# sieste/greb-climate-model

Measured on AMD Instinct MI355X. Metric: simulated-years/sec at 96x48 grid (ensemble aggregate); diffusion HBM GB/s vs roofline, higher is better.
Workload: dtype f32; 1 GPU; 96x48 GREB ensemble, 512 members/GPU x 1 GPU, CO2 sweep 280-1120 ppm, 32 scenario years after 1 flux-correction year, dt=12h, dt_crcl=0.5h; members_per_gpu=512, arithmetic=fast, gather=none (1 GPU)

## Files before the change

greb_climate_model_amd/csrc/greb_member.hip:

```cpp
#include <cstdlib>

#include "greb_kernels.h"
#include "greb_pair.h"
#include "greb_physics_step.h"
#include "greb_stencil.h"

namespace greb {

constexpr int NX = 96, NY = 48, NQ = 24, NP = 4608;
constexpr int kThreads = 512;
constexpr int RS = 2 * NX + 16;
constexpr int XB = (NY + 2) * RS;
constexpr int kOffX = RS;
constexpr int kOffW = 2 * XB + RS;
constexpr int kOffWX = 3 * XB;
constexpr int kOffWY = kOffWX + NP;
constexpr int kOffRowK = kOffWY + NP;
constexpr int kRowKCsDif = 7;
constexpr int kLdsFloats = kOffRowK + NY * kRowKWords;
constexpr size_t kLdsBytes = (size_t)kLdsFloats * sizeof(float);

bool member_layout_supported(const RowTables& t, int nx, int ny) {
  if (nx != NX || ny != NY) return false;
  for (int k = 0; k < NY; ++k) {
    const bool sub = (k <= 9 || k >= 38);
    if ((t.subcycled[k] != 0) != sub) return false;
    const bool chain = (k == 0 || k == NY - 1);
    if ((t.dif_time2[k] > 1 || t.adv_time2[k] > 1) != chain) return false;
  }
  if (t.dif_time2[0] != t.dif_time2[NY - 1] || t.adv_time2[0] != t.adv_time2[NY - 1]) return false;
  return true;
}

__device__ __forceinline__ f4 comp(const q8& q, int tr) {
  return tr == 0 ? f4{{q.v[0].x, q.v[1].x, q.v[2].x, q.v[3].x}} : f4{{q.v[0].y, q.v[1].y, q.v[2].y, q.v[3].y}};
}
__device__ __forceinline__ q8 zip(const f4& a, const f4& b) {
  q8 r;
#pragma unroll
  for (int i = 0; i < 4; ++i) r.v[i] = v2{a.v[i], b.v[i]};
  return r;
}

struct TaskAddr { int c, l, r, kq; };

__device__ __forceinline__ q8 ld8p(const lfloat* p) {
  const vfloat4 a = *(const __attribute__((address_space(3))) vfloat4*)p;
  const vfloat4 b = *(const __attribute__((address_space(3))) vfloat4*)(p + kHalfRow);
  q8 r;
  r.v[0] = v2{a.x, a.y}; r.v[1] = v2{a.z, a.w}; r.v[2] = v2{b.x, b.y}; r.v[3] = v2{b.z, b.w};
  return r;
}

template <bool SUB>
__device__ __forceinline__ q8 fast_row(const q8& LT, const q8& CT, const q8& RT, const q8& Tm2, const q8& Tm1, const q8& Tp1,
                                       const q8& Tp2, const q8& LW, const q8& CW, const q8& RW, const q8& Wm2, const q8& Wm1,
                                       const q8& Wp1, const q8& Wp2, const f4& xq, const f4& yq, bool last_quad,
                                       float cs_dif, float dif_ccy, bool calm_q) {
  v2 T[12], w[12];
#pragma unroll
  for (int j = 0; j < 4; ++j) {
    T[j] = LT.v[j]; T[4 + j] = CT.v[j]; T[8 + j] = RT.v[j];
    w[j] = LW.v[j]; w[4 + j] = CW.v[j]; w[8 + j] = RW.v[j];
  }
  float um[4], up[4], vm[4], vp[4];
#pragma unroll
  for (int i = 0; i < 4; ++i) {
    split_sign(xq.v[i], um[i], up[i]);
    split_sign(yq.v[i], vm[i], vp[i]);
  }
  return substep_pair<SUB>(T, w, Tm2, Tm1, Tp1, Tp2, Wm2, Wm1, Wp1, Wp2, um, up, vm, vp, cs_dif, dif_ccy, last_quad, calm_q);
}

__device__ __forceinline__ void st8p(lfloat* o, const q8& xn) {
  vfloat4 a, b;
  a.x = xn.v[0].x; a.y = xn.v[0].y; a.z = xn.v[1].x; a.w = xn.v[1].y;
  b.x = xn.v[2].x; b.y = xn.v[2].y; b.z = xn.v[3].x; b.w = xn.v[3].y;
  *(__attribute__((address_space(3))) vfloat4*)o = a;
  *(__attribute__((address_space(3))) vfloat4*)(o + kHalfRow) = b;
}

__device__ __forceinline__ q8 strict_row(const q8& LT, const q8& CT, const q8& RT, const q8& Tm2, const q8& Tm1, const q8& Tp1,
                                         const q8& Tp2, const q8& LW, const q8& CW, const q8& RW, const q8& Wm2, const q8& Wm1,
                                         const q8& Wp1, const q8& Wp2, const f4& xq, const f4& yq, int k, int q,
                                         const RowK& rk, bool calm_q) {
#pragma clang fp contract(off)
  q8 xn;
  v2 T[12], w[12];
#pragma unroll
  for (int j = 0; j < 4; ++j) {
    T[j] = LT.v[j]; T[4 + j] = CT.v[j]; T[8 + j] = RT.v[j];
    w[j] = LW.v[j]; w[4 + j] = CW.v[j]; w[8 + j] = RW.v[j];
  }
  v2 dTx[4], dTy[4], dd[4], da[4];
  dif_lon_strict(T, w, rk.dif_cc, dTx);
  if (rk.sub) {
    v2 T1h[4] = {T[4], T[5], T[6], T[7]};
    clamp_add(T1h, dTx);
#pragma unroll
    for (int i = 0; i < 4; ++i) dTx[i] = T1h[i] - T[4 + i];
  }
  dif_lat_strict(CT, Tm1, Tp1, Wm1, Wp1, rk.dif_ccy, k, NY, dTy);
#pragma unroll
  for (int i = 0; i < 4; ++i) dd[i] = CW.v[i] * (dTx[i] + dTy[i]);
  if (!rk.sub) {
    adv_lon_full_strict(T, w, xq.v, rk.adv_cc, dTx);
  } else {
    v2 T1h[4] = {T[4], T[5], T[6], T[7]};
    adv_lon_sub_strict(T, w, xq.v, rk.adv_cc, q == NQ - 1, dTx);
    clamp_add(T1h, dTx);
#pragma unroll
    for (int i = 0; i < 4; ++i) dTx[i] = T1h[i] - T[4 + i];
  }
  adv_lat_strict(CT, Tm2, Tm1, Tp1, Tp2, Wm2, Wm1, Wp1, Wp2, yq.v, rk.adv_ccy, k, NY, dTy);
#pragma unroll
  for (int i = 0; i < 4; ++i) {
    da[i] = dTx[i] + dTy[i];
    const v2 xd = T[4 + i] + dd[i];
    v2 x = xd + da[i];
    if (calm_q) x.y = xd.y;
    xn.v[i] = x;
  }
  return xn;
}

template <bool STRICT, bool SUB>
__device__ __forceinline__ q8 one_row(const q8& LT, const q8& CT, const q8& RT, const q8& Tm2, const q8& Tm1, const q8& Tp1,
                                      const q8& Tp2, const q8& LW, const q8& CW, const q8& RW, const q8& Wm2, const q8& Wm1,
                                      const q8& Wp1, const q8& Wp2, const f4& xq, const f4& yq, int k, int q, const RowK& rk,
                                      bool calm_q) {
  if (STRICT) return strict_row(LT, CT, RT, Tm2, Tm1, Tp1, Tp2, LW, CW, RW, Wm2, Wm1, Wp1, Wp2, xq, yq, k, q, rk, calm_q);
  return fast_row<SUB>(LT, CT, RT, Tm2, Tm1, Tp1, Tp2, LW, CW, RW, Wm2, Wm1, Wp1, Wp2, xq, yq, q == NQ - 1, rk.dif_cc, rk.dif_ccy,
                       calm_q);
}

template <bool STRICT>
__device__ __forceinline__ RowK task_consts(const lfloat* lds, int k, float ccy_dif) {
  if (STRICT) return row_consts((const lfloat*)(lds + kOffRowK), k);
  RowK rk{};
  rk.dif_cc = lds[kOffRowK + k * kRowKWords + kRowKCsDif];
  rk.dif_ccy = ccy_dif;
  return rk;
}

template <bool STRICT, bool SUB>
__device__ __forceinline__ void row_task(lfloat* lds, int cur, const TaskAddr& ta, float ccy_dif, bool calm_q = false) {
  const int k = ta.kq & 255, q = ta.kq >> 8;
  const lfloat* Xc = lds + kOffX + cur * XB;
  const lfloat* Wc = lds + kOffW;
  const RowK rk = task_consts<STRICT>(lds, k, ccy_dif);
  const f4 xq = ld4(lds + kOffWX + k * NX + 4 * q), yq = ld4(lds + kOffWY + k * NX + 4 * q);
  const lfloat* xb = Xc + ta.c - 2 * RS;
  const lfloat* wb = Wc + ta.c - 2 * RS;
  const q8 Tm2 = ld8p(xb), Tm1 = ld8p(xb + RS), CT = ld8p(xb + 2 * RS), Tp1 = ld8p(xb + 3 * RS), Tp2 = ld8p(xb + 4 * RS);
  const q8 Wm2 = ld8p(wb), Wm1 = ld8p(wb + RS), CW = ld8p(wb + 2 * RS), Wp1 = ld8p(wb + 3 * RS), Wp2 = ld8p(wb + 4 * RS);
  const q8 LT = ld8p(Xc + ta.l), RT = ld8p(Xc + ta.r), LW = ld8p(Wc + ta.l), RW = ld8p(Wc + ta.r);
  const q8 xn = one_row<STRICT, SUB>(LT, CT, RT, Tm2, Tm1, Tp1, Tp2, LW, CW, RW, Wm2, Wm1, Wp1, Wp2, xq, yq, k, q, rk, calm_q);
  st8p(lds + kOffX + (cur ^ 1) * XB + ta.c, xn);
}

template <bool STRICT, bool SUB>
__device__ __forceinline__ void row_task2(lfloat* lds, int cur, const TaskAddr& ta, float ccy_dif, bool calm_q = false) {
  const int k = ta.kq & 255, q = ta.kq >> 8;
  const lfloat* Xc = lds + kOffX + cur * XB;
  const lfloat* Wc = lds + kOffW;
  const lfloat* xb = Xc + ta.c - 2 * RS;
  const lfloat* wb = Wc + ta.c - 2 * RS;
  const q8 T0 = ld8p(xb), T1 = ld8p(xb + RS), T2 = ld8p(xb + 2 * RS), T3 = ld8p(xb + 3 * RS), T4 = ld8p(xb + 4 * RS);
  const q8 W0 = ld8p(wb), W1 = ld8p(wb + RS), W2 = ld8p(wb + 2 * RS), W3 = ld8p(wb + 3 * RS), W4 = ld8p(wb + 4 * RS);
  lfloat* out = lds + kOffX + (cur ^ 1) * XB + ta.c;
  {
    const q8 LT = ld8p(Xc + ta.l), RT = ld8p(Xc + ta.r), LW = ld8p(Wc + ta.l), RW = ld8p(Wc + ta.r);
    const f4 xq = ld4(lds + kOffWX + k * NX + 4 * q), yq = ld4(lds + kOffWY + k * NX + 4 * q);
    const RowK rk = task_consts<STRICT>(lds, k, ccy_dif);
    st8p(out, one_row<STRICT, SUB>(LT, T2, RT, T0, T1, T3, T4, LW, W2, RW, W0, W1, W3, W4, xq, yq, k, q, rk, calm_q));
  }
  __builtin_amdgcn_sched_barrier(0);
  {
    const q8 T5 = ld8p(xb + 5 * RS), W5 = ld8p(wb + 5 * RS);
    const q8 LT = ld8p(Xc + ta.l + RS), RT = ld8p(Xc + ta.r + RS), LW = ld8p(Wc + ta.l + RS), RW = ld8p(Wc + ta.r + RS);
    const f4 xq = ld4(lds + kOffWX + (k + 1) * NX + 4 * q), yq = ld4(lds + kOffWY + (k + 1) * NX + 4 * q);
    const RowK rk = task_consts<STRICT>(lds, k + 1, ccy_dif);
    st8p(out + RS, one_row<STRICT, SUB>(LT, T3, RT, T1, T2, T4, T5, LW, W3, RW, W1, W2, W4, W5, xq, yq, k + 1, q, rk, calm_q));
  }
}

struct BulkTasks { TaskAddr t[3]; };

enum { kNone = 0, kS1 = 1, kF1 = 2, kST = 3, kFT = 4 };
struct Pass { int kind, index; };
__host__ __device__ constexpr Pass deal_fast(int wave, int i) {
  constexpr Pass none{kNone, 0};
#if defined(GREB_TUNING) && defined(GREB_DEAL_FAST)
  constexpr Pass t[8][3] = {GREB_DEAL_FAST};
#else
  constexpr Pass t[8][3] = {
       {{kST, 0}, {kF1, 0}, none},      {{kST, 2}, {kF1, 1}, none},
       {{kFT, 1}, {kF1, 3}, none},      {{kFT, 2}, {kS1, 0}, {kF1, 2}},
       {{kST, 1}, none, none},          {{kFT, 0}, none, none},
       {none, none, none},              {{kF1, 4}, none, none}};
#endif
  return t[wave][i];
}
__host__ __device__ constexpr Pass deal_strict(int wave, int i) {
  constexpr Pass none{kNone, 0};
  constexpr Pass t[8][3] = {
       {{kST, 0}, {kFT, 0}, none},      {{kST, 2}, {kF1, 0}, {kF1, 1}},
       {none, none, none},              {none, none, none},
       {{kST, 1}, none, none},          {{kF1, 2}, {kF1, 3}, none},
       {{kFT, 1}, {kS1, 0}, none},      {{kFT, 2}, {kF1, 4}, none}};
  return t[wave][i];
}
template <bool STRICT>
__host__ __device__ constexpr Pass deal(int wave, int i) { return STRICT ? deal_strict(wave, i) : deal_fast(wave, i); }
#if defined(GREB_TUNING) && defined(GREB_POLAR_WAVE_FAST)
constexpr int kPolarWaveFast = GREB_POLAR_WAVE_FAST;
#else
constexpr int kPolarWaveFast = 6;
#endif
template <bool STRICT>
__host__ __device__ constexpr bool is_polar_wave(int wave) { return STRICT ? (wave == 2 || wave == 3) : wave == kPolarWaveFast; }

struct RowQuad { int k, q, valid; };
__host__ __device__ constexpr int task_rows(int kind) { return kind == kST || kind == kFT ? 2 : (kind == kS1 || kind == kF1 ? 1 : 0); }
__host__ __device__ constexpr RowQuad task_rowquad(int kind, int t) {
  int k = 1, q = 0, valid = 0;
  const int r = t / NQ;
  q = t % NQ;
  if (kind == kST) { valid = r < 8; k = r < 4 ? 1 + 2 * r : (r == 4 ? 41 : (r == 5 ? 39 : (r == 6 ? 45 : 43))); }
  else if (kind == kFT) { valid = r < 8; k = 10 + 2 * r; }
  else if (kind == kS1) { valid = r < 2; k = r == 0 ? 9 : 38; if (r == 1) q = (q + 4) % NQ; }
  else if (kind == kF1) { valid = r < 12; k = r < 6 ? 26 + 2 * r : 27 + 2 * (r - 6); }
  if (!valid) { k = 1; q = 0; }
  return RowQuad{k, q, valid};
}

__host__ __device__ constexpr int kind_passes(int kind) { return kind == kST || kind == kFT ? 3 : (kind == kS1 ? 1 : (kind == kF1 ? 5 : 0)); }
__host__ __device__ constexpr int pass_tasks(int kind, int index) {
  const int total = kind == kST || kind == kFT ? 8 * NQ : (kind == kS1 ? 2 * NQ : (kind == kF1 ? 12 * NQ : 0));
  const int left = total - 64 * index;
  return left >= 64 ? 64 : (left > 0 ? left : 0);
}

struct DealCover { int n[NY * NQ]; };
template <bool STRICT>
__host__ __device__ constexpr DealCover deal_cover() {
  DealCover c{};
  for (int w = 0; w < 8; ++w)
    for (int i = 0; i < 3; ++i) {
      const Pass p = deal<STRICT>(w, i);
      if (p.kind == kNone) continue;
      for (int lane = 0; lane < 64; ++lane) {
        const RowQuad rq = task_rowquad(p.kind, 64 * p.index + lane);
        for (int j = 0; j < (rq.valid ? task_rows(p.kind) : 0); ++j) ++c.n[(rq.k + j) * NQ + rq.q];
      }
    }
  return c;
}
template <bool STRICT>
__host__ __device__ constexpr bool deal_is_complete() {
  for (int w = 0; w < 8; ++w)
    for (int i = 0; i < 3; ++i) {
      const Pass p = deal<STRICT>(w, i);
      if (is_polar_wave<STRICT>(w) && p.kind != kNone) return false;
      if (p.kind != kNone && (p.index < 0 || p.index >= kind_passes(p.kind))) return false;
    }
  const DealCover c = deal_cover<STRICT>();
  for (int k = 0; k < NY; ++k)
    for (int q = 0; q < NQ; ++q) if (c.n[k * NQ + q] != (k >= 1 && k <= NY - 2 ? 1 : 0)) return false;
  return true;
}
static_assert(deal_is_complete<true>() && deal_is_complete<false>(),
              "a deal must compute every row-quad of rows 1 .. 46 exactly once and give the polar waves no bulk pass");

void member_deal_cover(bool strict, int* counts) {
  constexpr DealCover cs = deal_cover<true>(), cf = deal_cover<false>();
  for (int i = 0; i < NY * NQ; ++i) counts[i] = strict ? cs.n[i] : cf.n[i];
}

template <bool STRICT>
__device__ __forceinline__ BulkTasks make_tasks(int wave, int lane) {
  BulkTasks b;
#pragma unroll
  for (int i = 0; i < 3; ++i) {
    const RowQuad rq = task_rowquad(deal<STRICT>(wave, i).kind, deal<STRICT>(wave, i).index * 64 + lane);
    const int k = rq.k, q = rq.q, valid = rq.valid;
    TaskAddr a;
    a.c = k * RS + 4 * q;
    a.l = k * RS + 4 * (q == 0 ? NQ - 1 : q - 1);
    a.r = k * RS + 4 * (q == NQ - 1 ? 0 : q + 1);
    a.kq = valid ? (k | (q << 8)) : -1;
    asm volatile("" : "+v"(a.c), "+v"(a.l), "+v"(a.r), "+v"(a.kq));
    b.t[i] = a;
  }
  return b;
}

template <bool STRICT, int SLOT, int I>
__device__ __forceinline__ void bulk_task(lfloat* lds, int cur, const BulkTasks& tasks, float ccy_dif, int dbg, bool calm_q) {
  constexpr int kind = deal<STRICT>(SLOT, I).kind, ntask = pass_tasks(kind, deal<STRICT>(SLOT, I).index);
  if constexpr (kind != kNone && ntask > 0) {
    if (ntask < 64 && tasks.t[I].kq < 0) return;
    if constexpr (kind == kS1) { if (!(dbg & 1)) row_task<STRICT, true>(lds, cur, tasks.t[I], ccy_dif, calm_q); }
    else if constexpr (kind == kF1) { if (!(dbg & 2)) row_task<STRICT, false>(lds, cur, tasks.t[I], ccy_dif, calm_q); }
    else if constexpr (kind == kST) { if (!(dbg & 1)) row_task2<STRICT, true>(lds, cur, tasks.t[I], ccy_dif, calm_q); }
    else { if (!(dbg & 2)) row_task2<STRICT, false>(lds, cur, tasks.t[I], ccy_dif, calm_q); }
  }
}
template <bool STRICT, int SLOT>
__device__ __forceinline__ void bulk_substep(lfloat* lds, int cur, const BulkTasks& tasks, float ccy_dif, int dbg,
                                             bool calm_q = false) {
  bulk_task<STRICT, SLOT, 0>(lds, cur, tasks, ccy_dif, dbg, calm_q);
  bulk_task<STRICT, SLOT, 1>(lds, cur, tasks, ccy_dif, dbg, calm_q);
  bulk_task<STRICT, SLOT, 2>(lds, cur, tasks, ccy_dif, dbg, calm_q);
}

__device__ __forceinline__ int pair_off(int l) { return (l & 1) * kHalfRow + (l >> 1) * 4; }
__device__ __forceinline__ void load_win10(const lfloat* row, int l, v2 t[10]) {
  const int lm2 = l >= 2 ? l - 2 : l + 46, lm1 = l >= 1 ? l - 1 : 47, lp1 = l <= 46 ? l + 1 : 0, lp2 = l <= 45 ? l + 2 : l - 46;
  const int idx[5] = {lm2, lm1, l, lp1, lp2};
#pragma unroll
  for (int i = 0; i < 5; ++i) {
    const vfloat4 a = *(const __attribute__((address_space(3))) vfloat4*)(row + pair_off(idx[i]));
    t[2 * i] = v2{a.x, a.y}; t[2 * i + 1] = v2{a.z, a.w};
  }
}
__device__ __forceinline__ void st_pair2(lfloat* p, v2 a, v2 b) {
  vfloat4 x; x.x = a.x; x.y = a.y; x.z = b.x; x.w = b.y;
  *(__attribute__((address_space(3))) vfloat4*)p = x;
}

__device__ __forceinline__ void chain_substep_strict(lfloat* lds, int cur, int pole, int l , bool calm_q = false) {
  if (l >= 48) return;
  const int k = pole ? NY - 1 : 0;
  const RowK rk = row_consts((const lfloat*)(lds + kOffRowK), k);
  const lfloat* Xc = lds + kOffX + cur * XB;
  const lfloat* Wc = lds + kOffW;
  v2 T0w[10], w[10];
  load_win10(Xc + k * RS, l, T0w);
  load_win10(Wc + k * RS, l, w);
  const float u0 = lds[kOffWX + k * NX + 2 * l], u1 = lds[kOffWX + k * NX + 2 * l + 1];
  const float v0 = lds[kOffWY + k * NX + 2 * l], v1 = lds[kOffWY + k * NX + 2 * l + 1];
  const int k1 = pole ? k - 1 : k + 1, k2 = pole ? k - 2 : k + 2;
  v2 T1[2], T2[2], W1[2], W2[2];
  {
    const vfloat4 a = *(const __attribute__((address_space(3))) vfloat4*)(Xc + k1 * RS + pair_off(l));
    const vfloat4 b = *(const __attribute__((address_space(3))) vfloat4*)(Xc + k2 * RS + pair_off(l));
    const vfloat4 c = *(const __attribute__((address_space(3))) vfloat4*)(Wc + k1 * RS + pair_off(l));
    const vfloat4 d = *(const __attribute__((address_space(3))) vfloat4*)(Wc + k2 * RS + pair_off(l));
    T1[0] = v2{a.x, a.y}; T1[1] = v2{a.z, a.w}; T2[0] = v2{b.x, b.y}; T2[1] = v2{b.z, b.w};
    W1[0] = v2{c.x, c.y}; W1[1] = v2{c.z, c.w}; W2[0] = v2{d.x, d.y}; W2[1] = v2{d.z, d.w};
  }
  const v2 own[2] = {T0w[4], T0w[5]};
  const bool bug_lane = (l == 46);
  const int am2 = 4 * (l >= 2 ? l - 2 : l + 46), am1 = 4 * (l >= 1 ? l - 1 : 47), ap1 = 4 * (l <= 46 ? l + 1 : 0),
            ap2 = 4 * (l <= 45 ? l + 2 : l - 46);
  auto from = [](int addr, v2 x) {
    return v2{__int_as_float(__builtin_amdgcn_ds_bpermute(addr, __float_as_int(x.x))),
              __int_as_float(__builtin_amdgcn_ds_bpermute(addr, __float_as_int(x.y)))};
  };
  const float uu[2] = {u0, u1};

  v2 Th[2][2];
#pragma unroll
  for (int which = 0; which < 2; ++which) {
    const int time2 = __builtin_amdgcn_readfirstlane(which ? rk.adv_time2 : rk.dif_time2);
    const float cc = which ? rk.adv_cc : rk.dif_cc;
    v2 T[10];
#pragma unroll
    for (int i = 0; i < 10; ++i) T[i] = T0w[i];
    v2 th[2] = {own[0], own[1]};
    for (int tt = 0; tt < time2; ++tt) {
      if (tt > 0) {
        T[1] = from(am2, th[1]); T[2] = from(am1, th[0]); T[3] = from(am1, th[1]);
        T[4] = th[0]; T[5] = th[1];
        T[6] = from(ap1, th[0]); T[7] = from(ap1, th[1]); T[8] = from(ap2, th[0]);
      }
#pragma unroll
      for (int pt = 0; pt < 2; ++pt) {
#pragma clang fp contract(off)
        const int c = 4 + pt;
        v2 dd;
        if (which) dd = adv_lon_sub_point_strict(T, w, uu[pt], cc, c, bug_lane && pt == 1);
        else dd = div20(cc * dif_S_strict(T, w, c));
        dd = clamp_e(dd, T[c]);
        th[pt] = T[c] + dd;
      }
    }
    Th[which][0] = th[0]; Th[which][1] = th[1];
  }

  v2 xn[2];
  const float vv[2] = {v0, v1};
#pragma unroll
  for (int pt = 0; pt < 2; ++pt) {
#pragma clang fp contract(off)
    const v2 t0 = own[pt], w0 = w[4 + pt], a1 = T1[pt], a2 = T2[pt], b1 = W1[pt], b2 = W2[pt];
    const float vm = split_m(vv[pt]), vp = split_p(vv[pt]);
    v2 dTy, aTy;
    if (pole == 0) {
      dTy = rk.dif_ccy * b1 * (-t0 + a1);
      aTy = div3(rk.adv_ccy * (vp * (b1 * (t0 - a1) + b2 * (t0 - a2))));
    } else {
      dTy = rk.dif_ccy * b1 * (a1 - t0);
      aTy = div3(rk.adv_ccy * (-vm * (b1 * (t0 - a1) + b2 * (t0 - a2))));
    }
    const v2 dd = w0 * ((Th[0][pt] - t0) + dTy);
    const v2 da = (Th[1][pt] - t0) + aTy;
    const v2 xd = t0 + dd;
    v2 x = xd + da;
    if (calm_q) x.y = xd.y;
    xn[pt] = x;
  }
  st_pair2(lds + kOffX + (cur ^ 1) * XB + k * RS + pair_off(l), xn[0], xn[1]);
}

struct QuadChain {
  ChainK kd, ka;
  float w0[6], W1[6], W2[6];
  float own[6];
  float cv[6];
  float ccy;
  int at[3];
  int row[3];
  int time2_dif, time2_adv;
  bool calm;
};

__device__ __forceinline__ void quad_chain_setup(const lfloat* lds, int cur, int lane, bool calm_q, QuadChain& c) {
  const int r = lane >> 4, j = lane & 15, pole = r >> 1, C = r & 1;
  const int k = pole ? NY - 1 : 0, k1 = pole ? k - 1 : k + 1, k2 = pole ? k - 2 : k + 2;
  const RowK rk = row_consts((const lfloat*)(lds + kOffRowK), k);
  c.time2_dif = rk.dif_time2; c.time2_adv = rk.adv_time2; c.ccy = rk.dif_ccy;
  c.calm = calm_q && C == 1;
  c.row[0] = k * RS; c.row[1] = k1 * RS; c.row[2] = k2 * RS;
#pragma unroll
  for (int t = 0; t < 3; ++t) c.at[t] = pair_off(3 * j + t) + C;
  const lfloat* Wc = lds + kOffW;
  float w[12];
  static_for<12>([&](auto I) {
    constexpr int i = I;
    int x = 6 * j - 3 + i;
    x = x < 0 ? x + NX : (x >= NX ? x - NX : x);
    w[i] = Wc[c.row[0] + pair_off(x >> 1) + (x & 1) * 2 + C];
  });
  const float third = rk.adv_ccy * (1.f / 3.f), csd = rk.dif_cc * 0.05f, csa = rk.adv_cc * 0.05f;
  float Kd[6][6], Ka[6][6];
  static_for<6>([&](auto I) {
    constexpr int i = I, p = 3 + i;
    const int o = c.at[i >> 1] + (i & 1) * 2;
    c.w0[i] = w[p];
    c.own[i] = lds[kOffX + cur * XB + c.row[0] + o];
    c.W1[i] = Wc[c.row[1] + o];
    c.W2[i] = Wc[c.row[2] + o];
    const float u = lds[kOffWX + k * NX + 6 * j + i], v = lds[kOffWY + k * NX + 6 * j + i];
    c.cv[i] = pole == 0 ? third * fminf(v, 0.f) : -third * fmaxf(v, 0.f);
    Kd[i][0] = -csd * w[p - 3]; Kd[i][1] = (-3.f * csd) * w[p - 2]; Kd[i][2] = (-6.f * csd) * w[p - 1];
    Kd[i][3] = (6.f * csd) * w[p + 1]; Kd[i][4] = (3.f * csd) * w[p + 2]; Kd[i][5] = csd * w[p + 3];
    const float um = csa * fmaxf(u, 0.f), up = csa * fminf(u, 0.f);
    Ka[i][0] = -um * w[p - 3]; Ka[i][1] = (-4.f * um) * w[p - 2]; Ka[i][2] = (-10.f * um) * w[p - 1];
    Ka[i][3] = (-10.f * up) * w[p + 1]; Ka[i][4] = (-4.f * up) * w[p + 2]; Ka[i][5] = -up * w[p + 3];
    if (i == 3 && j == 15) {
      Ka[i][4] = -up * w[p + 3]; Ka[i][5] = -up * w[p + 3];
    }
  });
  c.kd = chain_pack(Kd);
  c.ka = chain_pack(Ka);
}

__device__ __forceinline__ void quad_chain_substep(lfloat* lds, int cur, QuadChain& c) {
  const lfloat* Xc = lds + kOffX + cur * XB;
  float own[6], T1[6], T2[6];
#pragma unroll
  for (int i = 0; i < 6; ++i) {
    const int o = c.at[i >> 1] + (i & 1) * 2;
    own[i] = c.own[i];
    T1[i] = Xc[c.row[1] + o];
    T2[i] = Xc[c.row[2] + o];
  }
  float Td[6], Ta[6];
#pragma unroll
  for (int i = 0; i < 6; ++i) { Td[i] = own[i]; Ta[i] = own[i]; }
  chain_run6<true>(Td, c.kd, c.time2_dif);
  chain_run6<true>(Ta, c.ka, c.time2_adv);
  lfloat* out = lds + kOffX + (cur ^ 1) * XB + c.row[0];
#pragma unroll
  for (int i = 0; i < 6; ++i) {
    const float g1 = c.W1[i] * (T1[i] - own[i]);
    const float d2 = c.W2[i] * (own[i] - T2[i]);
    const float ddy = c.ccy * g1;
    const float day = c.cv[i] * (d2 - g1);
    const float dd = c.w0[i] * ((Td[i] - own[i]) + ddy);
    float da = (Ta[i] - own[i]) + day;
    if (c.calm) da = 0.f;
    c.own[i] = (own[i] + dd) + da;
    out[c.at[i >> 1] + (i & 1) * 2] = c.own[i];
  }
}

template <bool STRICT, bool REMAT = false>
__device__ __forceinline__ void stage_winds(lfloat* lds, const float* __restrict__ u, const float* __restrict__ v,
                                            const RowTables* __restrict__ tab) {
  int tid0 = threadIdx.x;
  if (REMAT) asm volatile("" : "+v"(tid0));
  constexpr int kIt = (NP / 4 + kThreads - 1) / kThreads;
  f4 uq[kIt], vq[kIt];
#pragma unroll
  for (int j = 0; j < kIt; ++j) {
    const int i = min(tid0 + j * kThreads, NP / 4 - 1);
    uq[j] = ld4(u + 4 * i); vq[j] = ld4(v + 4 * i);
  }
#pragma unroll
  for (int j = 0; j < kIt; ++j) {
    const int i = tid0 + j * kThreads;
    if (i < NP / 4) {
      const int k = i / NQ;
      if (!(STRICT || k == 0 || k == NY - 1)) {
        const RowK rk = row_consts((const lfloat*)(lds + kOffRowK), k);
        const float cu = rk.sub ? rk.adv_cc * 0.05f : rk.adv_cc * (1.f / 3.f);
        const float cv = rk.adv_ccy * (1.f / 3.f);
#pragma unroll
        for (int e = 0; e < 4; ++e) { uq[j].v[e] *= cu; vq[j].v[e] *= cv; }
        if (k == 1 || k == NY - 2) {
#pragma unroll
          for (int e = 0; e < 4; ++e) {
            const float y = vq[j].v[e];
            vq[j].v[e] = (k == 1 ? y > 0.f : y < 0.f) ? 3.f * y : y;
          }
        }
      }
      st4(lds + kOffWX + 4 * i, uq[j]); st4(lds + kOffWY + 4 * i, vq[j]);
    }
  }
  (void)tab;
}

template <bool STRICT>
struct Circ {
  __device__ __forceinline__ void init(lfloat* lds, const float* wz_air, const float* wz_vapor,
                                       const RowTables* __restrict__ tab) {
    for (int i = threadIdx.x; i < 6 * RS; i += kThreads) {
      const int g = i / RS, o = i % RS;
      lds[(g >> 1) * XB + (g & 1) * (NY + 1) * RS + o] = 0.f;
    }
    stage_row_consts(lds + kOffRowK, *tab, 0, NY);
    if (!STRICT)
      for (int k = threadIdx.x; k < NY; k += blockDim.x)
        lds[kOffRowK + k * kRowKWords + kRowKCsDif] = lds[kOffRowK + k * kRowKWords] * 0.05f;
    for (int i = threadIdx.x; i < NP / 4; i += kThreads)
      st8(lds + kOffW + (i / NQ) * RS, i % NQ, zip(ld4(wz_air + 4 * i), ld4(wz_vapor + 4 * i)));
  }

  template <int WAVE, bool NOT_CALM>
  __device__ __forceinline__ void role_loop(lfloat* lds, int cur, int nsub, int lane, int dbg, bool calm_runtime
#ifdef GREB_TUNING
                                            , bool stamp, unsigned long long& busy
#endif
  ) {
    const bool calm_q = NOT_CALM ? false : calm_runtime;
    constexpr bool kPolar = is_polar_wave<STRICT>(WAVE);
    BulkTasks tasks;
    QuadChain quad;
    if constexpr (!kPolar) tasks = make_tasks<STRICT>(WAVE, lane);
    else if constexpr (!STRICT) quad_chain_setup(lds, cur, lane, calm_q, quad);
    float ccy_dif = 0.f;
    if constexpr (!kPolar && !STRICT) ccy_dif = __int_as_float(__builtin_amdgcn_readfirstlane(__float_as_int(lds[kOffRowK + 2])));
#pragma unroll 1
    for (int tt = 0; tt < nsub; ++tt) {
#ifdef GREB_TUNING
      const unsigned long long t0 = stamp ? __builtin_amdgcn_s_memtime() : 0;
#endif
      if constexpr (kPolar && STRICT) { if (!(dbg & 4)) chain_substep_strict(lds, cur, WAVE - 2, lane, calm_q); }
      else if constexpr (kPolar) { if (!(dbg & 4)) quad_chain_substep(lds, cur, quad); }
      else bulk_substep<STRICT, WAVE>(lds, cur, tasks, ccy_dif, dbg, calm_q);
#ifdef GREB_TUNING
      if (stamp) busy += __builtin_amdgcn_s_memtime() - t0;
#endif
      __syncthreads();
      cur ^= 1;
    }
  }
  __device__ __forceinline__ void substeps(lfloat* lds, int cur, int nsub, int dbg = 0, bool calm_q = false
#ifdef GREB_TUNING
                                           , bool stamp = false, unsigned long long* busy = nullptr
#endif
  ) {
    int lane = threadIdx.x & 63;
    asm volatile("" : "+v"(lane));
#ifdef GREB_TUNING
    unsigned long long b = 0;
#define GREB_ROLE(W) case W: if (!STRICT && !calm_q) role_loop<W, true>(lds, cur, nsub, lane, dbg, false, stamp, b); \
                             else role_loop<W, false>(lds, cur, nsub, lane, dbg, calm_q, stamp, b); break;
#else
#define GREB_ROLE(W) case W: if (!STRICT && !calm_q) role_loop<W, true>(lds, cur, nsub, lane, dbg, false); \
                             else role_loop<W, false>(lds, cur, nsub, lane, dbg, calm_q); break;
#endif
    switch (__builtin_amdgcn_readfirstlane(threadIdx.x >> 6)) {
      GREB_ROLE(0) GREB_ROLE(1) GREB_ROLE(2) GREB_ROLE(3) GREB_ROLE(4) GREB_ROLE(5) GREB_ROLE(6) GREB_ROLE(7)
    }
#undef GREB_ROLE
#ifdef GREB_TUNING
    if (busy) *busy += b;
#endif
  }
};

template <bool STRICT>
__global__ __launch_bounds__(kThreads) void circulation_g96_kernel(const float* __restrict__ Xin,
                                                                   const float* __restrict__ wz,
                                                                   const float* __restrict__ ug,
                                                                   const float* __restrict__ vg,
                                                                   float* __restrict__ dX,
                                                                   const RowTables* __restrict__ tab, int nsub,
                                                                   int dbg) {
  extern __shared__ __align__(16) float lds_raw[];
  lfloat* lds = (lfloat*)lds_raw;
  const size_t fo = (size_t)blockIdx.x * NP;
  Circ<STRICT> c;
  c.init(lds, wz + fo, wz + fo, tab);
  for (int i = threadIdx.x; i < NP / 4; i += kThreads) {
    const f4 x = ld4(Xin + fo + 4 * i);
    st8(lds + kOffX + (i / NQ) * RS, i % NQ, zip(x, x));
  }
  __syncthreads();
  stage_winds<STRICT>(lds, ug + fo, vg + fo, tab);
  __syncthreads();
  c.substeps(lds, 0, nsub, dbg);
  const int cur = nsub & 1;
  for (int i = threadIdx.x; i < NP / 4; i += kThreads) {
    const f4 a = comp(ld8(lds + kOffX + cur * XB + (i / NQ) * RS, i % NQ), 0), b = ld4(Xin + fo + 4 * i);
    st4(dX + fo + 4 * i, f4{{a.v[0] - b.v[0], a.v[1] - b.v[1], a.v[2] - b.v[2], a.v[3] - b.v[3]}});
  }
}

hipError_t launch_circulation_g96(const float* X, const float* wz, const float* u, const float* v, float* dX,
                                  const RowTables* tab_dev, int batch, int nsub, bool strict, hipStream_t s) {
  auto kern = strict ? circulation_g96_kernel<true> : circulation_g96_kernel<false>;
  hipError_t e = hipFuncSetAttribute(reinterpret_cast<const void*>(kern),
                                     hipFuncAttributeMaxDynamicSharedMemorySize, (int)kLdsBytes);
  if (e != hipSuccess) return e;
  hipLaunchKernelGGL(kern, dim3(batch), dim3(kThreads), kLdsBytes, s, X, wz, u, v, dX, tab_dev, nsub,
                     tuning_int("GREB_DEBUG_SKIP", 0));
  return hipGetLastError();
}

template <bool STRICT, bool FLUX, bool EXP, bool BUDGET = false>
__global__ __launch_bounds__(kThreads) void member_kernel(MemberArgs a) {
  extern __shared__ __align__(16) float lds_raw[];
  lfloat* lds = (lfloat*)lds_raw;
  const int m = blockIdx.x, tid = threadIdx.x;
  float* state = a.state + (size_t)m * 5 * NP;
  float* acc = a.acc + (size_t)m * 6 * NP;
  float* corr = a.corr + (size_t)a.corr_index[m] * 3 * kNT * NP;
  const RowTables* tab = a.tabs + a.tab_index[m];

#ifdef GREB_TUNING
  for (int i = 0; i < (a.dbg >> 8) * (m & 7); ++i) __builtin_amdgcn_s_sleep(16);
#endif
  Circ<STRICT> circ;
  circ.init(lds, a.wz_air, a.wz_vapor, tab);
  for (int i = tid; i < NP / 4; i += kThreads)
    st8(lds + kOffX + (i / NQ) * RS, i % NQ, zip(ld4(state + NP + 4 * i), ld4(state + 3 * NP + 4 * i)));
  int cur = 0;
  const unsigned xsw = EXP ? member_switches(a, m) : 0u;
  const int nsub = (EXP && (xsw & kXNoCirc)) ? 0 : a.nsub;
  const float co2_flux = FLUX ? (a.co2_flux_m ? a.co2_flux_m[m] : a.co2_flux) : 0.f;
  __syncthreads();
#ifdef GREB_TUNING
  const bool stamp = a.stamps != nullptr;
  unsigned long long st_wind = 0, st_circ = 0, st_busy = 0, st_phys = 0;
  const unsigned long long st_c0 = stamp ? __builtin_amdgcn_s_memtime() : 0, st_r0 = stamp ? __builtin_amdgcn_s_memrealtime() : 0;
#define GREB_STAMP(var) const unsigned long long var = stamp ? __builtin_amdgcn_s_memtime() : 0
#else
#define GREB_STAMP(var)
#endif

#pragma unroll 1
  for (int s = 0; s < a.nsteps; ++s) {
    const long long it = a.it0 + s;
    const StepClock ck = step_clock<FLUX>(a, it, NP);
    const int ityr = ck.ityr, yr_rel = ck.yr_rel;
    const size_t off = ck.off;

    GREB_STAMP(t_a);
    stage_winds<STRICT, EXP && !STRICT>(lds, a.uclim + off, a.vclim + off, tab);
    __syncthreads();
    GREB_STAMP(t_b);

#ifdef GREB_TUNING
    circ.substeps(lds, cur, nsub, 0, EXP && (xsw & kXQDiffOnly), stamp, &st_busy);
#else
    circ.substeps(lds, cur, nsub, 0, EXP && (xsw & kXQDiffOnly));
#endif
    cur ^= nsub & 1;
    GREB_STAMP(t_c);

    const Phys P = a.phys[m];
    const float co2 = FLUX ? co2_flux : a.co2[(size_t)m * a.co2_stride + a.co2_year0 + yr_rel];
    lfloat* Xf = lds + kOffX + cur * XB;
    lfloat* red = lds + kOffX + (cur ^ 1) * XB;
    if constexpr (BUDGET) {
      const BudgetSink bs = budget_sink<true>(a, m, ck);
#pragma unroll 1
      for (int qd = tid; qd < NP / 4; qd += kThreads) {
        const q8 xpair = ld8(Xf + (qd / NQ) * RS, qd % NQ);
        const PhysIn in = physics_load<FLUX, EXP>(a, qd, ck, state, acc, corr, xsw);
        (void)physics_compute<STRICT, FLUX, EXP, true>(a, P, in, co2, comp(xpair, 0), comp(xpair, 1), xsw, bs, 4 * qd);
      }
    }
#pragma unroll 1
    for (int qd = tid; qd < NP / 4; qd += kThreads) {
#ifdef GREB_TUNING
      if ((a.dbg & 4) && qd >= kThreads) break;
#endif
      const q8 xpair = ld8(Xf + (qd / NQ) * RS, qd % NQ);
      f4 oTa, oq, tsm;
      physics_quad<STRICT, FLUX, EXP>(a, P, m, qd, ck, co2, state, acc, corr, comp(xpair, 0), comp(xpair, 1), oTa, oq, tsm, xsw);
      st8(Xf + (qd / NQ) * RS, qd % NQ, zip(oTa, oq));
      if (ityr == kNT) st4(red + 4 * qd, tsm);
    }
    if (ityr == kNT) {
      __syncthreads();
      if (STRICT) {
        if (tid == 0 && a.yearly) {
#pragma clang fp contract(off)
          float sum = 0.f;
          for (int i = 0; i < NP; ++i) sum += red[i];
// ... 61 lines not shown
```

greb_climate_model_amd/csrc/greb_pair.h:

```cpp
#pragma once
#include "greb_device.h"

namespace greb {


constexpr int kHalfRow = 96;
struct q8 {
  v2 v[4];
};
__device__ __forceinline__ q8 ld8(const lfloat* row, int q) {
  const vfloat4 a = *(const __attribute__((address_space(3))) vfloat4*)(row + 4 * q);
  const vfloat4 b = *(const __attribute__((address_space(3))) vfloat4*)(row + kHalfRow + 4 * q);
  q8 r;
  r.v[0] = v2{a.x, a.y}; r.v[1] = v2{a.z, a.w}; r.v[2] = v2{b.x, b.y}; r.v[3] = v2{b.z, b.w};
  return r;
}
__device__ __forceinline__ void st8(lfloat* row, int q, const q8& x) {
  vfloat4 a, b;
  a.x = x.v[0].x; a.y = x.v[0].y; a.z = x.v[1].x; a.w = x.v[1].y;
  b.x = x.v[2].x; b.y = x.v[2].y; b.z = x.v[3].x; b.w = x.v[3].y;
  *(__attribute__((address_space(3))) vfloat4*)(row + 4 * q) = a;
  *(__attribute__((address_space(3))) vfloat4*)(row + kHalfRow + 4 * q) = b;
}
__device__ __forceinline__ q8 zero8() {
  q8 r;
  r.v[0] = r.v[1] = r.v[2] = r.v[3] = v2{0.f, 0.f};
  return r;
}

__device__ __forceinline__ v2 pk_sub(v2 a, v2 b) {
  v2 r;
  asm("v_pk_add_f32 %0, %1, %2 neg_lo:[0,1] neg_hi:[0,1]" : "=v"(r) : "v"(a), "v"(b));
  return r;
}
__device__ __forceinline__ void split_sign(float u, float& pos, float& neg) {
  pos = __builtin_amdgcn_fmed3f(u, 0.f, 3.0e38f);
  neg = u - pos;
}

struct Flux2 {
  v2 Pp[10];
  v2 Pm[10];
};

__device__ __forceinline__ void make_flux2(const v2 T[12], const v2 w[12], Flux2& f) {
#pragma unroll
  for (int m = 1; m <= 9; ++m) {
    const v2 e = T[m + 1] - T[m];
    if (m >= 4) f.Pp[m] = w[m + 1] * e;
    if (m <= 6) f.Pm[m] = w[m] * e;
  }
}

__device__ __forceinline__ void dif_lon2(const Flux2& f, float cs, v2 d[4]) {
#pragma unroll
  for (int i = 0; i < 4; ++i) {
    const int c = 4 + i;
    const v2 a = f.Pp[c] - f.Pm[c - 1], b = f.Pp[c + 1] - f.Pm[c - 2], g = f.Pp[c + 2] - f.Pm[c - 3];
    d[i] = cs * (6.f * a + (3.f * b + g));
  }
}

__device__ __forceinline__ void adv_lon_full2(const Flux2& f, const v2 T[12], const v2 w[12], const float um[4],
                                              const float up[4], v2 d[4]) {
#pragma unroll
  for (int i = 0; i < 4; ++i) {
    const int c = 4 + i;
    const v2 em2 = w[c - 2] * (T[c] - T[c - 2]), ep2 = w[c + 2] * (T[c] - T[c + 2]);
    d[i] = up[i] * (ep2 - f.Pp[c]) - um[i] * (f.Pm[c - 1] + em2);
  }
}

__device__ __forceinline__ void adv_lon_sub2(const Flux2& f, const v2 T[12], const v2 w[12], const float um[4],
                                             const float up[4], bool last_quad, v2 d[4]) {
#pragma unroll
  for (int i = 0; i < 4; ++i) {
    const int c = 4 + i;
    const v2 am = 10.f * f.Pm[c - 1] + (4.f * f.Pm[c - 2] + f.Pm[c - 3]);
    v2 ap = 10.f * f.Pp[c] + (4.f * f.Pp[c + 1] + f.Pp[c + 2]);
    if (i == 1) {
      const v2 bug = 10.f * f.Pp[c] - w[c + 3] * (T[c + 1] - T[c + 3]);
      ap = last_quad ? bug : ap;
    }
    d[i] = -up[i] * ap - um[i] * am;
  }
}

__device__ __forceinline__ void clamp_add2(v2 T1h[4], v2 d[4]) {
#pragma unroll
  for (int i = 0; i < 4; ++i) {
    v2 dd = d[i];
    dd.x = (dd.x <= -T1h[i].x) ? -0.9f * T1h[i].x : dd.x;
    dd.y = (dd.y <= -T1h[i].y) ? -0.9f * T1h[i].y : dd.y;
    d[i] = dd;
    T1h[i] = T1h[i] + dd;
  }
}

__device__ __forceinline__ void lat2(const v2 T0[4], const v2 Tm2[4], const v2 Tm1[4], const v2 Tp1[4],
                                     const v2 Tp2[4], const v2 wm2[4], const v2 wm1[4], const v2 wp1[4],
                                     const v2 wp2[4], const float vm[4], const float vp[4], float ccy_dif,
                                     v2 ddif[4], v2 dadv[4]) {
#pragma unroll
  for (int i = 0; i < 4; ++i) {
    const v2 gm1 = wm1[i] * pk_sub(Tm1[i], T0[i]), gp1 = wp1[i] * pk_sub(Tp1[i], T0[i]);
    const v2 dm2 = wm2[i] * pk_sub(T0[i], Tm2[i]), dp2 = wp2[i] * pk_sub(T0[i], Tp2[i]);
    ddif[i] = ccy_dif * (gm1 + gp1);
    dadv[i] = vp[i] * (dp2 - gp1) - vm[i] * (dm2 - gm1);
  }
}

template <bool SUB>
__device__ __forceinline__ q8 substep_pair(const v2 T[12], const v2 w[12], const q8& Tm2, const q8& Tm1,
                                           const q8& Tp1, const q8& Tp2, const q8& wm2, const q8& wm1,
                                           const q8& wp1, const q8& wp2, const float um[4], const float up[4],
                                           const float vm[4], const float vp[4], float cs_dif, float ccy_dif,
                                           bool last_quad, bool calm_q = false) {
  Flux2 f;
  make_flux2(T, w, f);
  v2 ddx[4], dax[4], ddy[4], day[4];
  dif_lon2(f, cs_dif, ddx);
  if (SUB) {
    adv_lon_sub2(f, T, w, um, up, last_quad, dax);
    v2 T1h[4], T2h[4];
#pragma unroll
    for (int i = 0; i < 4; ++i) { T1h[i] = T[4 + i] + ddx[i]; T2h[i] = T[4 + i] + dax[i]; }
    float mn = min3f(T1h[0].x, T1h[0].y, T1h[1].x);
    mn = min3f(mn, T1h[1].y, T1h[2].x); mn = min3f(mn, T1h[2].y, T1h[3].x); mn = min3f(mn, T1h[3].y, T2h[0].x);
    mn = min3f(mn, T2h[0].y, T2h[1].x); mn = min3f(mn, T2h[1].y, T2h[2].x); mn = min3f(mn, T2h[2].y, T2h[3].x);
    mn = min3f(mn, T2h[3].y, T2h[3].y);
    if (__builtin_expect(!(mn > 0.f), 0)) {
#pragma unroll
      for (int i = 0; i < 4; ++i) { T1h[i] = T[4 + i]; T2h[i] = T[4 + i]; }
      clamp_add2(T1h, ddx);
      clamp_add2(T2h, dax);
    }
#pragma unroll
    for (int i = 0; i < 4; ++i) { ddx[i] = T1h[i] - T[4 + i]; dax[i] = T2h[i] - T[4 + i]; }
  } else {
    adv_lon_full2(f, T, w, um, up, dax);
  }
  lat2(&T[4], Tm2.v, Tm1.v, Tp1.v, Tp2.v, wm2.v, wm1.v, wp1.v, wp2.v, vm, vp, ccy_dif, ddy, day);
  q8 r;
#pragma unroll
  for (int i = 0; i < 4; ++i) {
    const v2 dd = w[4 + i] * (ddx[i] + ddy[i]);
    v2 da = dax[i] + day[i];
    if (calm_q) da.y = 0.f;
    r.v[i] = (T[4 + i] + dd) + da;
  }
  return r;
}

}
```

Before: 5718 simulated-years/s.

## Precompute wind-sign ballot masks once and select upwind operands via cndmask

```diff
diff --git a/greb_climate_model_amd/csrc/greb_member.hip b/greb_climate_model_amd/csrc/greb_member.hip
--- a/greb_climate_model_amd/csrc/greb_member.hip
+++ b/greb_climate_model_amd/csrc/greb_member.hip
@@ -55,21 +55,15 @@
 template <bool SUB>
 __device__ __forceinline__ q8 fast_row(const q8& LT, const q8& CT, const q8& RT, const q8& Tm2, const q8& Tm1, const q8& Tp1,
                                        const q8& Tp2, const q8& LW, const q8& CW, const q8& RW, const q8& Wm2, const q8& Wm1,
-                                       const q8& Wp1, const q8& Wp2, const f4& xq, const f4& yq, bool last_quad,
-                                       float cs_dif, float dif_ccy, bool calm_q) {
+                                       const q8& Wp1, const q8& Wp2, const f4& xq, const f4& yq, const WindSigns& ws,
+                                       bool last_quad, float cs_dif, float dif_ccy, bool calm_q) {
   v2 T[12], w[12];
 #pragma unroll
   for (int j = 0; j < 4; ++j) {
     T[j] = LT.v[j]; T[4 + j] = CT.v[j]; T[8 + j] = RT.v[j];
     w[j] = LW.v[j]; w[4 + j] = CW.v[j]; w[8 + j] = RW.v[j];
   }
-  float um[4], up[4], vm[4], vp[4];
-#pragma unroll
-  for (int i = 0; i < 4; ++i) {
-    split_sign(xq.v[i], um[i], up[i]);
-    split_sign(yq.v[i], vm[i], vp[i]);
-  }
-  return substep_pair<SUB>(T, w, Tm2, Tm1, Tp1, Tp2, Wm2, Wm1, Wp1, Wp2, um, up, vm, vp, cs_dif, dif_ccy, last_quad, calm_q);
+  return substep_pair<SUB>(T, w, Tm2, Tm1, Tp1, Tp2, Wm2, Wm1, Wp1, Wp2, xq.v, ws.x, yq.v, ws.y, cs_dif, dif_ccy, last_quad, calm_q);
 }
 
 __device__ __forceinline__ void st8p(lfloat* o, const q8& xn) {
@@ -127,11 +121,11 @@
 template <bool STRICT, bool SUB>
 __device__ __forceinline__ q8 one_row(const q8& LT, const q8& CT, const q8& RT, const q8& Tm2, const q8& Tm1, const q8& Tp1,
                                       const q8& Tp2, const q8& LW, const q8& CW, const q8& RW, const q8& Wm2, const q8& Wm1,
-                                      const q8& Wp1, const q8& Wp2, const f4& xq, const f4& yq, int k, int q, const RowK& rk,
-                                      bool calm_q) {
+                                      const q8& Wp1, const q8& Wp2, const f4& xq, const f4& yq, const WindSigns& ws, int k, int q,
+                                      const RowK& rk, bool calm_q) {
   if (STRICT) return strict_row(LT, CT, RT, Tm2, Tm1, Tp1, Tp2, LW, CW, RW, Wm2, Wm1, Wp1, Wp2, xq, yq, k, q, rk, calm_q);
-  return fast_row<SUB>(LT, CT, RT, Tm2, Tm1, Tp1, Tp2, LW, CW, RW, Wm2, Wm1, Wp1, Wp2, xq, yq, q == NQ - 1, rk.dif_cc, rk.dif_ccy,
-                       calm_q);
+  return fast_row<SUB>(LT, CT, RT, Tm2, Tm1, Tp1, Tp2, LW, CW, RW, Wm2, Wm1, Wp1, Wp2, xq, yq, ws, q == NQ - 1, rk.dif_cc,
+                       rk.dif_ccy, calm_q);
 }
 
 template <bool STRICT>
@@ -144,7 +138,8 @@
 }
 
 template <bool STRICT, bool SUB>
-__device__ __forceinline__ void row_task(lfloat* lds, int cur, const TaskAddr& ta, float ccy_dif, bool calm_q = false) {
+__device__ __forceinline__ void row_task(lfloat* lds, int cur, const TaskAddr& ta, const WindSigns* ws, float ccy_dif,
+                                         bool calm_q = false) {
   const int k = ta.kq & 255, q = ta.kq >> 8;
   const lfloat* Xc = lds + kOffX + cur * XB;
   const lfloat* Wc = lds + kOffW;
@@ -155,12 +150,14 @@
   const q8 Tm2 = ld8p(xb), Tm1 = ld8p(xb + RS), CT = ld8p(xb + 2 * RS), Tp1 = ld8p(xb + 3 * RS), Tp2 = ld8p(xb + 4 * RS);
   const q8 Wm2 = ld8p(wb), Wm1 = ld8p(wb + RS), CW = ld8p(wb + 2 * RS), Wp1 = ld8p(wb + 3 * RS), Wp2 = ld8p(wb + 4 * RS);
   const q8 LT = ld8p(Xc + ta.l), RT = ld8p(Xc + ta.r), LW = ld8p(Wc + ta.l), RW = ld8p(Wc + ta.r);
-  const q8 xn = one_row<STRICT, SUB>(LT, CT, RT, Tm2, Tm1, Tp1, Tp2, LW, CW, RW, Wm2, Wm1, Wp1, Wp2, xq, yq, k, q, rk, calm_q);
+  const q8 xn = one_row<STRICT, SUB>(LT, CT, RT, Tm2, Tm1, Tp1, Tp2, LW, CW, RW, Wm2, Wm1, Wp1, Wp2, xq, yq, ws[0], k, q, rk,
+                                     calm_q);
   st8p(lds + kOffX + (cur ^ 1) * XB + ta.c, xn);
 }
 
 template <bool STRICT, bool SUB>
-__device__ __forceinline__ void row_task2(lfloat* lds, int cur, const TaskAddr& ta, float ccy_dif, bool calm_q = false) {
+__device__ __forceinline__ void row_task2(lfloat* lds, int cur, const TaskAddr& ta, const WindSigns* ws, float ccy_dif,
+                                          bool calm_q = false) {
   const int k = ta.kq & 255, q = ta.kq >> 8;
   const lfloat* Xc = lds + kOffX + cur * XB;
   const lfloat* Wc = lds + kOffW;
@@ -173,7 +170,7 @@
     const q8 LT = ld8p(Xc + ta.l), RT = ld8p(Xc + ta.r), LW = ld8p(Wc + ta.l), RW = ld8p(Wc + ta.r);
     const f4 xq = ld4(lds + kOffWX + k * NX + 4 * q), yq = ld4(lds + kOffWY + k * NX + 4 * q);
     const RowK rk = task_consts<STRICT>(lds, k, ccy_dif);
-    st8p(out, one_row<STRICT, SUB>(LT, T2, RT, T0, T1, T3, T4, LW, W2, RW, W0, W1, W3, W4, xq, yq, k, q, rk, calm_q));
+    st8p(out, one_row<STRICT, SUB>(LT, T2, RT, T0, T1, T3, T4, LW, W2, RW, W0, W1, W3, W4, xq, yq, ws[0], k, q, rk, calm_q));
   }
   __builtin_amdgcn_sched_barrier(0);
   {
@@ -181,11 +178,13 @@
     const q8 LT = ld8p(Xc + ta.l + RS), RT = ld8p(Xc + ta.r + RS), LW = ld8p(Wc + ta.l + RS), RW = ld8p(Wc + ta.r + RS);
     const f4 xq = ld4(lds + kOffWX + (k + 1) * NX + 4 * q), yq = ld4(lds + kOffWY + (k + 1) * NX + 4 * q);
     const RowK rk = task_consts<STRICT>(lds, k + 1, ccy_dif);
-    st8p(out + RS, one_row<STRICT, SUB>(LT, T3, RT, T1, T2, T4, T5, LW, W3, RW, W1, W2, W4, W5, xq, yq, k + 1, q, rk, calm_q));
+    st8p(out + RS,
+         one_row<STRICT, SUB>(LT, T3, RT, T1, T2, T4, T5, LW, W3, RW, W1, W2, W4, W5, xq, yq, ws[1], k + 1, q, rk, calm_q));
   }
 }
 
 struct BulkTasks { TaskAddr t[3]; };
+struct BulkSigns { WindSigns s[3][2]; };
 
 enum { kNone = 0, kS1 = 1, kF1 = 2, kST = 3, kFT = 4 };
 struct Pass { int kind, index; };
@@ -196,9 +195,9 @@
 #else
   constexpr Pass t[8][3] = {
        {{kST, 0}, {kF1, 0}, none},      {{kST, 2}, {kF1, 1}, none},
-       {{kFT, 1}, {kF1, 3}, none},      {{kFT, 2}, {kS1, 0}, {kF1, 2}},
+       {{kFT, 1}, {kF1, 3}, none},      {{kFT, 2}, {kS1, 0}, none},
        {{kST, 1}, none, none},          {{kFT, 0}, none, none},
-       {none, none, none},              {{kF1, 4}, none, none}};
+       {none, none, none},              {{kF1, 2}, {kF1, 4}, none}};
 #endif
   return t[wave][i];
 }
@@ -296,23 +295,44 @@
   return b;
 }
 
+template <int WAVE>
+__device__ __forceinline__ void make_signs(const lfloat* lds, const BulkTasks& tasks, BulkSigns& b) {
+  static_for<3>([&](auto I) {
+    constexpr int i = I, rows = task_rows(deal_fast(WAVE, i).kind);
+    if constexpr (rows > 0) {
+      const int kq = tasks.t[i].kq < 0 ? 1 : tasks.t[i].kq, k = kq & 255, q = kq >> 8;
+#pragma unroll
+      for (int j = 0; j < rows; ++j) {
+        const f4 xq = ld4(lds + kOffWX + (k + j) * NX + 4 * q), yq = ld4(lds + kOffWY + (k + j) * NX + 4 * q);
+#pragma unroll
+        for (int e = 0; e < 4; ++e) {
+          unsigned long long mx = __builtin_amdgcn_ballot_w64(xq.v[e] > 0.f), my = __builtin_amdgcn_ballot_w64(yq.v[e] > 0.f);
+          asm volatile("" : "+s"(mx), "+s"(my));
+          b.s[i][j].x[e] = mx; b.s[i][j].y[e] = my;
+        }
+      }
+    }
+  });
+}
+
 template <bool STRICT, int SLOT, int I>
-__device__ __forceinline__ void bulk_task(lfloat* lds, int cur, const BulkTasks& tasks, float ccy_dif, int dbg, bool calm_q) {
+__device__ __forceinline__ void bulk_task(lfloat* lds, int cur, const BulkTasks& tasks, const BulkSigns& signs, float ccy_dif,
+                                          int dbg, bool calm_q) {
   constexpr int kind = deal<STRICT>(SLOT, I).kind, ntask = pass_tasks(kind, deal<STRICT>(SLOT, I).index);
   if constexpr (kind != kNone && ntask > 0) {
     if (ntask < 64 && tasks.t[I].kq < 0) return;
-    if constexpr (kind == kS1) { if (!(dbg & 1)) row_task<STRICT, true>(lds, cur, tasks.t[I], ccy_dif, calm_q); }
-    else if constexpr (kind == kF1) { if (!(dbg & 2)) row_task<STRICT, false>(lds, cur, tasks.t[I], ccy_dif, calm_q); }
-    else if constexpr (kind == kST) { if (!(dbg & 1)) row_task2<STRICT, true>(lds, cur, tasks.t[I], ccy_dif, calm_q); }
-    else { if (!(dbg & 2)) row_task2<STRICT, false>(lds, cur, tasks.t[I], ccy_dif, calm_q); }
+    if constexpr (kind == kS1) { if (!(dbg & 1)) row_task<STRICT, true>(lds, cur, tasks.t[I], signs.s[I], ccy_dif, calm_q); }
+    else if constexpr (kind == kF1) { if (!(dbg & 2)) row_task<STRICT, false>(lds, cur, tasks.t[I], signs.s[I], ccy_dif, calm_q); }
+    else if constexpr (kind == kST) { if (!(dbg & 1)) row_task2<STRICT, true>(lds, cur, tasks.t[I], signs.s[I], ccy_dif, calm_q); }
+    else { if (!(dbg & 2)) row_task2<STRICT, false>(lds, cur, tasks.t[I], signs.s[I], ccy_dif, calm_q); }
   }
 }
 template <bool STRICT, int SLOT>
-__device__ __forceinline__ void bulk_substep(lfloat* lds, int cur, const BulkTasks& tasks, float ccy_dif, int dbg,
-                                             bool calm_q = false) {
-  bulk_task<STRICT, SLOT, 0>(lds, cur, tasks, ccy_dif, dbg, calm_q);
-  bulk_task<STRICT, SLOT, 1>(lds, cur, tasks, ccy_dif, dbg, calm_q);
-  bulk_task<STRICT, SLOT, 2>(lds, cur, tasks, ccy_dif, dbg, calm_q);
+__device__ __forceinline__ void bulk_substep(lfloat* lds, int cur, const BulkTasks& tasks, const BulkSigns& signs, float ccy_dif,
+                                             int dbg, bool calm_q = false) {
+  bulk_task<STRICT, SLOT, 0>(lds, cur, tasks, signs, ccy_dif, dbg, calm_q);
+  bulk_task<STRICT, SLOT, 1>(lds, cur, tasks, signs, ccy_dif, dbg, calm_q);
+  bulk_task<STRICT, SLOT, 2>(lds, cur, tasks, signs, ccy_dif, dbg, calm_q);
 }
 
 __device__ __forceinline__ int pair_off(int l) { return (l & 1) * kHalfRow + (l >> 1) * 4; }
@@ -560,9 +580,11 @@
     const bool calm_q = NOT_CALM ? false : calm_runtime;
     constexpr bool kPolar = is_polar_wave<STRICT>(WAVE);
     BulkTasks tasks;
+    BulkSigns signs;
     QuadChain quad;
     if constexpr (!kPolar) tasks = make_tasks<STRICT>(WAVE, lane);
     else if constexpr (!STRICT) quad_chain_setup(lds, cur, lane, calm_q, quad);
+    if constexpr (!kPolar && !STRICT) make_signs<WAVE>(lds, tasks, signs);
     float ccy_dif = 0.f;
     if constexpr (!kPolar && !STRICT) ccy_dif = __int_as_float(__builtin_amdgcn_readfirstlane(__float_as_int(lds[kOffRowK + 2])));
 #pragma unroll 1
@@ -572,7 +594,7 @@
 #endif
       if constexpr (kPolar && STRICT) { if (!(dbg & 4)) chain_substep_strict(lds, cur, WAVE - 2, lane, calm_q); }
       else if constexpr (kPolar) { if (!(dbg & 4)) quad_chain_substep(lds, cur, quad); }
-      else bulk_substep<STRICT, WAVE>(lds, cur, tasks, ccy_dif, dbg, calm_q);
+      else bulk_substep<STRICT, WAVE>(lds, cur, tasks, signs, ccy_dif, dbg, calm_q);
 #ifdef GREB_TUNING
       if (stamp) busy += __builtin_amdgcn_s_memtime() - t0;
 #endif
diff --git a/greb_climate_model_amd/csrc/greb_pair.h b/greb_climate_model_amd/csrc/greb_pair.h
--- a/greb_climate_model_amd/csrc/greb_pair.h
+++ b/greb_climate_model_amd/csrc/greb_pair.h
@@ -33,10 +33,22 @@
   asm("v_pk_add_f32 %0, %1, %2 neg_lo:[0,1] neg_hi:[0,1]" : "=v"(r) : "v"(a), "v"(b));
   return r;
 }
-__device__ __forceinline__ void split_sign(float u, float& pos, float& neg) {
-  pos = __builtin_amdgcn_fmed3f(u, 0.f, 3.0e38f);
-  neg = u - pos;
+template <bool NEG_A>
+__device__ __forceinline__ float wind_operand(float a, float b, unsigned long long pos) {
+  float r;
+  if (NEG_A) asm("v_cndmask_b32_e64 %0, -%1, -%2, %3" : "=v"(r) : "v"(a), "v"(b), "s"(pos));
+  else asm("v_cndmask_b32_e64 %0, %1, -%2, %3" : "=v"(r) : "v"(a), "v"(b), "s"(pos));
+  return r;
 }
+template <bool NEG_A = false>
+__device__ __forceinline__ v2 wind_term(float u, unsigned long long pos, v2 A, v2 B) {
+#pragma clang fp contract(off)
+  const v2 op{wind_operand<NEG_A>(A.x, B.x, pos), wind_operand<NEG_A>(A.y, B.y, pos)};
+  return u * op;
+}
+struct WindSigns {
+  unsigned long long x[4], y[4];
+};
 
 struct Flux2 {
   v2 Pp[10];
@@ -61,18 +73,18 @@
   }
 }
 
-__device__ __forceinline__ void adv_lon_full2(const Flux2& f, const v2 T[12], const v2 w[12], const float um[4],
-                                              const float up[4], v2 d[4]) {
+__device__ __forceinline__ void adv_lon_full2(const Flux2& f, const v2 T[12], const v2 w[12], const float u[4],
+                                              const unsigned long long pos[4], v2 d[4]) {
 #pragma unroll
   for (int i = 0; i < 4; ++i) {
     const int c = 4 + i;
     const v2 em2 = w[c - 2] * (T[c] - T[c - 2]), ep2 = w[c + 2] * (T[c] - T[c + 2]);
-    d[i] = up[i] * (ep2 - f.Pp[c]) - um[i] * (f.Pm[c - 1] + em2);
+    d[i] = wind_term(u[i], pos[i], ep2 - f.Pp[c], f.Pm[c - 1] + em2);
   }
 }
 
-__device__ __forceinline__ void adv_lon_sub2(const Flux2& f, const v2 T[12], const v2 w[12], const float um[4],
-                                             const float up[4], bool last_quad, v2 d[4]) {
+__device__ __forceinline__ void adv_lon_sub2(const Flux2& f, const v2 T[12], const v2 w[12], const float u[4],
+                                             const unsigned long long pos[4], bool last_quad, v2 d[4]) {
 #pragma unroll
   for (int i = 0; i < 4; ++i) {
     const int c = 4 + i;
@@ -82,7 +94,7 @@
       const v2 bug = 10.f * f.Pp[c] - w[c + 3] * (T[c + 1] - T[c + 3]);
       ap = last_quad ? bug : ap;
     }
-    d[i] = -up[i] * ap - um[i] * am;
+    d[i] = wind_term<true>(u[i], pos[i], ap, am);
   }
 }
 
@@ -99,29 +111,29 @@
 
 __device__ __forceinline__ void lat2(const v2 T0[4], const v2 Tm2[4], const v2 Tm1[4], const v2 Tp1[4],
                                      const v2 Tp2[4], const v2 wm2[4], const v2 wm1[4], const v2 wp1[4],
-                                     const v2 wp2[4], const float vm[4], const float vp[4], float ccy_dif,
+                                     const v2 wp2[4], const float v[4], const unsigned long long pos[4], float ccy_dif,
                                      v2 ddif[4], v2 dadv[4]) {
 #pragma unroll
   for (int i = 0; i < 4; ++i) {
     const v2 gm1 = wm1[i] * pk_sub(Tm1[i], T0[i]), gp1 = wp1[i] * pk_sub(Tp1[i], T0[i]);
     const v2 dm2 = wm2[i] * pk_sub(T0[i], Tm2[i]), dp2 = wp2[i] * pk_sub(T0[i], Tp2[i]);
     ddif[i] = ccy_dif * (gm1 + gp1);
-    dadv[i] = vp[i] * (dp2 - gp1) - vm[i] * (dm2 - gm1);
+    dadv[i] = wind_term(v[i], pos[i], dp2 - gp1, dm2 - gm1);
   }
 }
 
 template <bool SUB>
 __device__ __forceinline__ q8 substep_pair(const v2 T[12], const v2 w[12], const q8& Tm2, const q8& Tm1,
                                            const q8& Tp1, const q8& Tp2, const q8& wm2, const q8& wm1,
-                                           const q8& wp1, const q8& wp2, const float um[4], const float up[4],
-                                           const float vm[4], const float vp[4], float cs_dif, float ccy_dif,
+                                           const q8& wp1, const q8& wp2, const float u[4], const unsigned long long upos[4],
+                                           const float v[4], const unsigned long long vpos[4], float cs_dif, float ccy_dif,
                                            bool last_quad, bool calm_q = false) {
   Flux2 f;
   make_flux2(T, w, f);
   v2 ddx[4], dax[4], ddy[4], day[4];
   dif_lon2(f, cs_dif, ddx);
   if (SUB) {
-    adv_lon_sub2(f, T, w, um, up, last_quad, dax);
+    adv_lon_sub2(f, T, w, u, upos, last_quad, dax);
     v2 T1h[4], T2h[4];
 #pragma unroll
     for (int i = 0; i < 4; ++i) { T1h[i] = T[4 + i] + ddx[i]; T2h[i] = T[4 + i] + dax[i]; }
@@ -138,9 +150,9 @@
 #pragma unroll
     for (int i = 0; i < 4; ++i) { ddx[i] = T1h[i] - T[4 + i]; dax[i] = T2h[i] - T[4 + i]; }
   } else {
-    adv_lon_full2(f, T, w, um, up, dax);
+    adv_lon_full2(f, T, w, u, upos, dax);
   }
-  lat2(&T[4], Tm2.v, Tm1.v, Tp1.v, Tp2.v, wm2.v, wm1.v, wp1.v, wp2.v, vm, vp, ccy_dif, ddy, day);
+  lat2(&T[4], Tm2.v, Tm1.v, Tp1.v, Tp2.v, wm2.v, wm1.v, wp1.v, wp2.v, v, vpos, ccy_dif, ddy, day);
   q8 r;
 #pragma unroll
   for (int i = 0; i < 4; ++i) {
```

Result: faster. 5816 simulated-years/s, median of 6 (+1.7%).
